# patngnw/NewsRecommendation

Measured on AMD Instinct MI355X. Metric: train impressions/sec @ batch 512, NRMS, higher is better.
Workload: dtype bf16; 1 GPU; NRMS train step (fwd+bwd+Adam), MIND-small shapes: title_len=30, history=50, npratio=4, 300-d word table; per_gpu_batch=512, global_batch=512, vocab_rows=30000, freeze_embedding=False, compact_history=False, dense_batch=False, feed=resident, deterministic=False, optimizer=flat bucket + HIP fused Adam, parallelism=dp1

## Files before the change

newsrecommendation_amd/csrc/nr_api.hip:

```cpp
#include <stdarg.h>
#include <stdio.h>
#include <stdlib.h>
#include <string.h>

#include "nr_gemm.h"

int nr_launch_attn(bool bwd, int dtype, const void* qkv, const float* mask, void* y, const void* dy, void* dqkv, int n, int L,
                   int heads, int d_head, const DropCfg& drop, hipStream_t stream, const uint32_t* tmask = nullptr,
                   const float* bias = nullptr, const int32_t* seq_list = nullptr, const int32_t* seq_count = nullptr,
                   const int32_t* needed = nullptr);
bool nr_attn_pad_ok(int dtype, int L, int d_head, const void* p0, const void* p1);
bool nr_attn_rowsub_ok(int dtype, int L, int d_head, int heads);
bool nr_attn_compact_ok(int dtype, int L, int d_head, int heads);
int nr_launch_attn_bwd_compact(const void* qkv, const float* mask, const void* dy, void* dqkv, int n, int L, int heads, int d_head,
                               const DropCfg& drop, hipStream_t stream, const uint32_t* tmask, const float* bias, const int32_t* seq_list,
                               const int32_t* seq_count, const int32_t* pos, void* dump, float* db, const int32_t* nzf);
int nr_launch_attn_gather_fwd(const void* proj_table, const int32_t* ids, const float* mask, void* y, int n, int L, int heads,
                              int d_head, const DropCfg& drop, hipStream_t stream);
int nr_launch_pool_core_fwd(int dtype, const void* x, const void* e, const float* w2, const float* b2, const float* mask,
                            float* alpha, float* out, int ld_out, int n, int L, int N, int q, hipStream_t s,
                            const int32_t* needed = nullptr);
int nr_launch_pool_core_bwd(int dtype, const void* x, const void* e, const float* w2, const float* alpha, const float* g,
                            int ld_g, void* dpre, float* partial, float* dw2, float* db2, int n, int L, int N, int q,
                            hipStream_t s, const int32_t* seq_nz = nullptr);
// ... 939 lines not shown
  NR_CHECK_ARG(d != nullptr, "additive_pool: null descriptor");
  NR_CHECK_ARG(dtype_ok(d->dtype), "additive_pool: bad dtype %d", d->dtype);
  const int ch = nr_chunk(d->dtype);
  NR_CHECK_ARG(d->n >= 0 && d->L >= 1 && d->L <= 128 && d->N >= 1 && d->q >= 1, "additive_pool: bad shape n=%d L=%d N=%d q=%d", d->n, d->L,
               d->N, d->q);
  NR_CHECK_ARG(d->N % ch == 0 && d->q % ch == 0, "additive_pool: N=%d and q=%d must be multiples of %d for this dtype", d->N, d->q, ch);
  NR_CHECK_ARG(d->ldw1 >= d->N, "additive_pool: ldw1=%d < N=%d", d->ldw1, d->N);
  NR_CHECK_ARG(d->n == 0 || (d->x && d->w1 && d->b1 && d->w2 && d->b2), "additive_pool: null operand");
  return NR_OK;
}

int nr_additive_pool_fwd(const nr_pool_desc* d, void* e, float* alpha, float* out, int ld_out, nr_stream_t stream) {
  int rc = pool_check(d);
  if (rc) return rc;
  if (d->n == 0) return NR_OK;
  NR_CHECK_ARG(e && alpha && out && ld_out >= d->N, "additive_pool_fwd: null output / ld_out");
  NR_DEVICE_GUARD(stream, out);
  hipStream_t s = (hipStream_t)stream;
  if (nr_pool_fused_fwd_ok(d->dtype, d->n, d->L, d->N, d->q, d->ldw1) && ((((uintptr_t)d->x) | ((uintptr_t)d->w1) | ((uintptr_t)e)) & 15) == 0 &&
      d->N % 8 == 0 && d->mask == nullptr)
    return nr_launch_pool_fused_fwd(d->x, d->N, d->w1, d->ldw1, d->b1, d->w2, d->b2, d->mask, e, d->q, alpha, out, ld_out, d->n, d->L, d->N, d->q,
                                    d->seq_needed, s);
  RowSrc A = dense_rows(d->x, d->N, d->N);
  EpiArgs ep = store_epi(e, d->q, d->dtype, d->b1, 1);
  ep.seq_nz = d->seq_needed; ep.L = d->L;
  if ((rc = nr_launch_gemm_nt(d->dtype, A, d->w1, d->ldw1, d->n * d->L, d->q, d->N, EPI_STORE, ep, s))) return rc;
  return nr_launch_pool_core_fwd(d->dtype, d->x, e, d->w2, d->b2, d->mask, alpha, out, ld_out, d->n, d->L, d->N, d->q, s, d->seq_needed);
}

int nr_additive_pool_bwd(const nr_pool_desc* d, const void* e, const float* alpha, const float* g, int ld_g, const void* w1_t,
                         int ldw1t, void* dpre, float* partial, float* dw1, float* db1, float* dw2, float* db2, void* dx,
                         nr_stream_t stream) {
  int rc = pool_check(d);
  if (rc) return rc;
  if (d->n == 0) return NR_OK;
  NR_CHECK_ARG(e && alpha && g && dpre && partial && dw1 && db1 && dw2 && db2, "additive_pool_bwd: null operand");
  NR_DEVICE_GUARD(stream, dpre);
  NR_CHECK_ARG(d->partial_bytes >= pool_ws_elems(d->n, d->L, d->q, d->N, d->dtype) * sizeof(float),
               "additive_pool_bwd: partial holds %zu bytes, nr_pool_workspace_bytes() asks for %zu", d->partial_bytes,
               pool_ws_elems(d->n, d->L, d->q, d->N, d->dtype) * sizeof(float));
  float* tn_scratch = partial + pool_ws_ints(d->n, d->L, d->q);
  const size_t tn_floats = pool_tn_floats(d->n, d->L, d->q, d->N, d->dtype);
  hipStream_t s = (hipStream_t)stream;
  const int M = d->n * d->L;
  DetScope det(s);
  det.add(dw1, (size_t)d->q * d->N);
  det.add(db1, (size_t)d->q);
  det.add(dw2, (size_t)d->q);
  det.add(db2, 1);
  if ((rc = det.begin(true, true))) return rc;
  int32_t* ws = nullptr;
  if (pool_has_flags(d)) {
    ws = reinterpret_cast<int32_t*>(partial + pool_ws_used(d->n, d->q));
    if ((rc = nr_launch_row_flags_f32(g, ld_g, d->N, d->n, ws, s))) return rc;
  }
  const int32_t* zero_flags = ws != nullptr ? ws : d->seq_needed;
  if (ws != nullptr && dx != nullptr && w1_t != nullptr && !det.on() && nr_pool_fused_bwd_ok(d->dtype, d->n, d->L, d->N, d->q, ldw1t) && ld_g % 4 == 0 &&
      ((((uintptr_t)d->x) | ((uintptr_t)e) | ((uintptr_t)w1_t) | ((uintptr_t)dpre) | ((uintptr_t)dx) | ((uintptr_t)g)) & 15) == 0 && d->N % 8 == 0) {
    int rows = 0;
    if ((rc = nr_launch_pool_fused_bwd(d->x, d->N, e, d->q, alpha, g, ld_g, d->w2, w1_t, ldw1t, dpre, d->q, dx, d->N, partial,
                                       nr_pool_partial_rows(d->n), ws, d->n, d->L, d->N, d->q, s, &rows, d->dx_far_unwritten)))
      return rc;
    if ((rc = nr_launch_colsum_split(partial, rows, d->q + 1, d->q + 1, dw2, d->q, db2, s))) return rc;
    if ((rc = nr_launch_live_slabs(ws, d->n, d->L, s))) return rc;
    return gemm_tn_live_slabs(ws, d->n, dpre, d->q, d->x, d->N, dw1, d->N, db1, M, d->q, d->N, d->q, d->N, s, 0, tn_scratch, tn_floats);
  }
  if ((rc = nr_launch_pool_core_bwd(d->dtype, d->x, e, d->w2, alpha, g, ld_g, dpre, partial, dw2, db2, d->n, d->L, d->N, d->q, s, zero_flags)))
    return rc;
  RowSrc X = dense_rows(d->x, d->N, d->N);
  if (ws != nullptr) {
    if ((rc = nr_launch_live_slabs(ws, d->n, d->L, s))) return rc;
    if ((rc = gemm_tn_live_slabs(ws, d->n, dpre, d->q, d->x, d->N, dw1, d->N, db1, M, d->q, d->N, d->q, d->N, s, 0, tn_scratch, tn_floats))) return rc;
  } else if ((rc = nr_launch_gemm_tn(d->dtype, dpre, d->q, X, dw1, d->N, db1, M, d->q, d->N, d->q, d->N, s))) {
    return rc;
  }
  if (dx != nullptr) {
    NR_CHECK_ARG(w1_t != nullptr && ldw1t >= d->q, "additive_pool_bwd: w1_t [N, >=q] needed for dx");
    RowSrc P = dense_rows(dpre, d->q, d->q);
    EpiArgs ep = store_epi(dx, d->N, d->dtype, nullptr, 0);
    ep.rowscale = alpha; ep.G = g; ep.ldg = ld_g; ep.L = d->L;
    ep.seq_nz = zero_flags;
    rc = nr_launch_gemm_nt(d->dtype, P, w1_t, ldw1t, M, d->N, d->q, EPI_POOLBWD, ep, s);
  }
  return rc;
}

static int linear_rows(const nr_linear_desc* d, RowSrc* out) {
  NR_CHECK_ARG(d != nullptr, "linear: null descriptor");
  NR_CHECK_ARG(dtype_ok(d->dtype), "linear: bad dtype %d", d->dtype);
  const int ch = nr_chunk(d->dtype);
  NR_CHECK_ARG(d->M >= 0 && d->K >= 1 && d->N >= 1, "linear: bad shape M=%d K=%d N=%d", d->M, d->K, d->N);
  NR_CHECK_ARG(d->ldx >= round_up(d->K, ch) && d->ldw >= round_up(d->K, ch), "linear: ldx=%d / ldw=%d must cover K=%d rounded up to %d",
               d->ldx, d->ldw, d->K, ch);
  NR_CHECK_ARG(d->M == 0 || (d->x && d->w), "linear: null operand");
  RowSrc s = dense_rows(d->x, d->ldx, d->K);
  if (d->src_kind == NR_SRC_GATHER) {
    NR_CHECK_ARG(d->ids != nullptr && d->ids_stride >= 1, "linear: gather source without ids");
    s.kind = ROWS_GATHER; s.ids = d->ids; s.ids_stride = d->ids_stride;
  } else {
    NR_CHECK_ARG(d->src_kind == NR_SRC_DENSE, "linear: bad src_kind %d", d->src_kind);
  }
  *out = s;
  return NR_OK;
}

int nr_linear_fwd(const nr_linear_desc* d, float* out, int ld_out, nr_stream_t stream) {
  RowSrc A;
  int rc = linear_rows(d, &A);
  if (rc) return rc;
  if (d->M == 0) return NR_OK;
  NR_CHECK_ARG(out != nullptr && ld_out >= d->N, "linear_fwd: null output / ld_out");
  NR_DEVICE_GUARD(stream, out);
  EpiArgs ep = store_epi(out, ld_out, NR_F32, d->bias, 0);
  return nr_launch_gemm_nt(d->dtype, A, d->w, d->ldw, d->M, d->N, round_up(d->K, nr_chunk(d->dtype)), EPI_STORE, ep, (hipStream_t)stream);
}

int nr_linear_bwd(const nr_linear_desc* d, const float* dout, int ld_dout, void* dout_ws, float* dw, float* db, float* dtable,
                  nr_stream_t stream) {
  RowSrc A;
  int rc = linear_rows(d, &A);
  if (rc) return rc;
  if (d->M == 0) return NR_OK;
  NR_CHECK_ARG(dout && dout_ws && dw && db, "linear_bwd: null operand");
  NR_DEVICE_GUARD(stream, dw);
// ... 27 lines not shown
```

newsrecommendation_amd/csrc/nr_gemm.h:

```cpp
#pragma once
#include "nr_common.h"

enum { ROWS_DENSE = 0, ROWS_GATHER = 1, ROWS_IM2COL3 = 2 };

struct RowSrc {
  const void* base;
  const int32_t* ids;
  int ld;
  int ids_stride;
  int kind;
  int Tlen;
  int Dtrue;
  DropCfg drop;
  int gap;
};

enum {
  EPI_STORE = 0,
  EPI_POOLBWD = 1,
  EPI_SCATTER = 2,
  EPI_STORE_TANH = 3,
};

struct EpiArgs {
  void* C;
  int ldc;
  int out_dtype;
  const float* bias;
  int act_tanh;
  const float* rowscale;
  const float* G;
  int ldg, L;
  const int32_t* ids;
  int ids_stride;
  int Dtrue;
  DropCfg drop;
  const int32_t* row_count;
  const int32_t* row_idx;
  const int32_t* row_ids;
  const int32_t* seq_nz;
  void* rows_out;
  int ld_rows_out;
  int a_gap;
  const int32_t* a_idx;
  int a_dense;
  int tail_cus;
};

int nr_launch_gemm_nt(int dtype, const RowSrc& A, const void* B, int ldb, int M, int N, int K, int epi,
                      const EpiArgs& ep, hipStream_t stream);
int nr_launch_conv_rows(int dtype, const RowSrc& A, void* out, int n, hipStream_t stream, const int32_t* needed = nullptr, int margin = 0);
int nr_launch_rows_materialize(int dtype, const RowSrc& A, void* out, int ldo, int M, int K, hipStream_t stream,
                               const int32_t* needed = nullptr, int margin = 0, int L = 0, const int32_t* keep_all = nullptr);
int nr_launch_compact_rows(const int32_t* ids, int ids_stride, int M, int32_t* ws, hipStream_t stream);
int nr_launch_sort_rows_by_id(const int32_t* count, const int32_t* rows, const int32_t* ids, int Mmax, int table_rows, int32_t* hist,
                              int32_t* rows_out, int32_t* ids_out, hipStream_t stream, int32_t* k_out = nullptr,
                              int32_t* counted_cursor = nullptr);
int nr_launch_compact_rows_fwd(const int32_t* ids, int M, int n, int L, const void* table_row0, int cols, int32_t* ws,
                               hipStream_t stream, int32_t* posmap = nullptr, int32_t* zero4 = nullptr, int32_t* zhist = nullptr,
                               int nhist = 0);
int nr_launch_bias_rows(void* C, int ldc, int N, const float* bias, const int32_t* rows, const int32_t* count, int max_rows,
                        const uint32_t* tmask, int L, hipStream_t stream);
int nr_launch_title_flags(const void* dy, int n, int L, int N, int32_t* title_nz, hipStream_t stream);
int nr_launch_row_flags_f32(const float* g, int ld, int N, int n, int32_t* nz, hipStream_t stream);
int nr_launch_live_slabs(int32_t* ws, int n, int L, hipStream_t stream);
int nr_launch_needed_list(const int32_t* flags, int n, int32_t* out, void* y, size_t seq_bytes, hipStream_t stream, int reach = -1,
                          bool zeroed = false);
int nr_launch_seq_list(const int32_t* title_nz, const uint32_t* tmask, int n, int L, int32_t* out, hipStream_t stream, int reach = -1,
                       bool zeroed = false);
int nr_launch_zero_tail_rows(void* buf, int ld, const int32_t* count, int Mmax, hipStream_t stream, int32_t* za = nullptr, int na = 0,
                             int32_t* zb = nullptr, int nb = 0);
int nr_launch_gemm_tn_slabs(const void* dC, int ldc, const void* X, int ldx, float* dW, int ldw, float* db, int M, int N, int K,
                            int Nstore, int Kstore, const int32_t* slab_list, const int32_t* slab_count, hipStream_t stream, int xgap = 0,
                            float* scratch = nullptr, size_t scratch_floats = 0);
size_t nr_gemm_tn_scratch_floats(int M, int N, int K);
bool nr_gemm_tn_slabs_ok(int ldc, int ldx, int M, int N, int K);
int nr_pool_fused_fwd_ok(int dtype, int n, int L, int N, int q, int ldw1);
int nr_launch_pool_fused_fwd(const void* x, int ldx, const void* w1, int ldw1, const float* b1, const float* w2, const float* b2,
                             const float* mask, void* e, int lde, float* alpha, float* out, int ld_out, int n, int L, int N, int q,
                             const int32_t* needed, hipStream_t stream);
int nr_launch_gemm_tn_counted(const void* dC, int ldc, const void* X, int ldx, float* dW, int ldw, int Mmax, int N, int K, int Nstore,
                              int Kstore, const int32_t* row_count, hipStream_t stream, float* scratch = nullptr, size_t scratch_floats = 0);
int nr_pool_fused_bwd_ok(int dtype, int n, int L, int N, int q, int ldw1t);
int nr_launch_pool_fused_bwd(const void* x, int ldx, const void* e, int lde, const float* alpha, const float* g, int ldg, const float* w2,
                             const void* w1t, int ldw1t, void* dpre, int ldp, void* dx, int lddx, float* partial, int partial_rows,
                             const int32_t* nz, int n, int L, int N, int q, hipStream_t stream, int* grid_out, int dx_far_unwritten = 0);
int nr_launch_gather_live_rows(int dtype, const RowSrc& A, void* out, int ldo, int Mmax, int K, const int32_t* count, const int32_t* rows,
                               const int32_t* ids, hipStream_t stream, int32_t* hist = nullptr, int V = 0);
int nr_launch_gemm_tn(int dtype, const void* dC, int ldc, const RowSrc& A, float* dW, int ldw, float* db,
                      int M, int N, int K, int Nstore, int Kstore, hipStream_t stream);
int nr_launch_conv_table_live(const int32_t* ids, int ids_stride, const int32_t* seq_nz, int n, int T, int V, int32_t* hdr, int32_t* live_s,
                              int32_t* live_id, hipStream_t stream);
int nr_launch_conv_table_stage(int dtype, const void* dy, int n, int T, int N, const int32_t* hdr, const int32_t* live_s, bool compact, void* out,
                               int32_t* ident, hipStream_t stream);
int nr_launch_conv_table_rank(const int32_t* hdr, const int32_t* sort_s, const int32_t* sort_id, const int32_t* sort_k, const int32_t* cursor,
                              bool compact, int n, int32_t* ord_s, int32_t* ord_slot, hipStream_t stream);
int nr_launch_conv_table_scatter(int dx_dtype, const void* dx, int ldx, int n, int T, int D, int V, const int32_t* hdr, const int32_t* sort_id,
                                 const int32_t* cursor, const int32_t* ord_s, const int32_t* ord_slot, DropCfg drop, float* dtable,
                                 hipStream_t stream);
```

newsrecommendation_amd/csrc/nr_gemm.hip:

```cpp
#include <stdlib.h>

#include "nr_gemm.h"
#include "nr_scatter_tail.h"

namespace {

constexpr int BM = 128, BN = 128, BK = 32, NTHR = 256;
constexpr int SC = BN + 4;

template <typename T> struct TileCfg {
  static constexpr int CH = 16 / (int)sizeof(T);
  static constexpr int SK = BK + CH;
  static constexpr int CPR = BK / CH;
  static constexpr int NCH = BM * CPR / NTHR;
  static constexpr int RPC = BM / CH;
  static constexpr size_t STAGE_BYTES = (size_t)2 * 2 * BM * SK * sizeof(T);
};
constexpr size_t EPI_BYTES = (size_t)64 * SC * sizeof(float);

template <typename T> constexpr size_t smem_bytes() {
  return TileCfg<T>::STAGE_BYTES > EPI_BYTES ? TileCfg<T>::STAGE_BYTES : EPI_BYTES;
}

union Chunk {
// ... 3280 lines not shown
      for (int u = 0; u < 8; ++u) {
        const int t = base + u * 1024 + tid;
        if (t < n) sFlag[t] = v[u] != 0 ? 1 : 0;
      }
    }
    __syncthreads();
  }
  const int per = (nslab + 1023) / 1024, s0 = tid * per, s1 = min(nslab, s0 + per);
  const int tq = s0 < nslab ? (32 * s0) / L : 0, rq = 32 * s0 - tq * L;
  auto flag = [&](int t) { return in_lds ? (int)sFlag[t] : (title_nz[t] != 0 ? 1 : 0); };
  auto walk = [&](auto&& emit) {
    int t = tq, rem = rq;
    for (int s = s0; s < s1; ++s) {
      int lv = flag(min(t, n - 1)), e = rem + 31, te = t;
      while (e >= L) {
        e -= L; ++te;
        if (te < n) lv |= flag(te);
      }
      emit(s, lv != 0);
      rem += 32;
      while (rem >= L) { rem -= L; ++t; }
    }
  };
  int c = 0;
  walk([&](int, bool lv) { c += lv ? 1 : 0; });
  const int lane = tid & 63, wv = tid >> 6;
  int v = c;
#pragma unroll
  for (int o = 1; o < 64; o <<= 1) {
    const int t = __shfl_up(v, o, 64);
    if (lane >= o) v += t;
  }
  if (lane == 63) sCnt[wv] = v;
  __syncthreads();
  if (wv == 0) {
    int w = lane < 16 ? sCnt[lane] : 0;
#pragma unroll
    for (int o = 1; o < 16; o <<= 1) {
      const int t = __shfl_up(w, o, 64);
      if (lane >= o) w += t;
    }
    if (lane < 16) sCnt[16 + lane] = w;
  }
  __syncthreads();
  int pos = v - c + (wv > 0 ? sCnt[16 + wv - 1] : 0);
  walk([&](int s, bool lv) { if (lv) list[pos++] = s; });
  if (tid == 1023) sCnt[1023] = sCnt[16 + 15];
  if (tid == 1023) *count = sCnt[1023];
}
}

namespace {
__global__ __launch_bounds__(256) void slab_flags_kernel(const int32_t* __restrict__ title_nz, int n, int L, int nslab,
                                                         unsigned char* __restrict__ flags) {
  const int s = blockIdx.x * 256 + threadIdx.x;
  if (s >= nslab) return;
  const int t0 = (32 * s) / L, t1 = min(n - 1, (32 * s + 31) / L);
  bool lv = false;
  for (int t = t0; t <= t1; ++t) lv |= title_nz[t] != 0;
  flags[s] = lv ? 1 : 0;
}
__global__ __launch_bounds__(1024) void slab_list_kernel(const unsigned char* __restrict__ flags, int nslab, int32_t* __restrict__ count,
                                                         int32_t* __restrict__ list) {
  __shared__ int sCnt[32];
  extern __shared__ __attribute__((aligned(16))) unsigned char sFlag[];
  const int tid = threadIdx.x, lane = tid & 63, wv = tid >> 6;
  const int words = (nslab + 3) / 4;
  const uint32_t* fw = reinterpret_cast<const uint32_t*>(flags);
  for (int base = 0; base < words; base += 8 * 1024) {
    uint32_t v[8];
#pragma unroll
    for (int u = 0; u < 8; ++u) {
      const int w = base + u * 1024 + tid;
      v[u] = w < words ? fw[w] : 0u;
    }
#pragma unroll
    for (int u = 0; u < 8; ++u) {
      const int w = base + u * 1024 + tid;
      if (w < words) reinterpret_cast<uint32_t*>(sFlag)[w] = v[u];
    }
  }
  __syncthreads();
  const int per = (nslab + 1023) / 1024, s0 = tid * per, s1 = min(nslab, s0 + per);
  int c = 0;
  for (int s2 = s0; s2 < s1; ++s2) c += sFlag[s2];
  int v = c;
#pragma unroll
  for (int o = 1; o < 64; o <<= 1) {
    const int t = __shfl_up(v, o, 64);
    if (lane >= o) v += t;
  }
  if (lane == 63) sCnt[wv] = v;
  __syncthreads();
  if (wv == 0) {
    int w = lane < 16 ? sCnt[lane] : 0;
#pragma unroll
    for (int o = 1; o < 16; o <<= 1) {
      const int t = __shfl_up(w, o, 64);
      if (lane >= o) w += t;
    }
    if (lane < 16) sCnt[16 + lane] = w;
  }
  __syncthreads();
  int pos = v - c + (wv > 0 ? sCnt[16 + wv - 1] : 0);
  for (int s2 = s0; s2 < s1; ++s2)
    if (sFlag[s2]) list[pos++] = s2;
  if (tid == 0) *count = sCnt[16 + 15];
}
// ... 97 lines not shown
}
__global__ __launch_bounds__(256) void zero_unneeded_kernel(const int32_t* __restrict__ flags, uint4* __restrict__ y, int chunks16, int n,
                                                            int reach) {
  const int seq = blockIdx.x;
  if (flags[seq] != 0) return;
  if (reach >= 0) {
    bool near = false;
    for (int t = max(0, seq - reach) + (int)threadIdx.x; t <= min(n - 1, seq + reach); t += 256) near |= flags[t] != 0;
    if (!__syncthreads_or(near)) return;
  }
  uint4* p = y + (size_t)seq * chunks16;
  for (int c = threadIdx.x; c < chunks16; c += 256) p[c] = make_uint4(0, 0, 0, 0);
}
}
int nr_launch_needed_list(const int32_t* flags, int n, int32_t* out, void* y, size_t seq_bytes, hipStream_t stream, int reach, bool zeroed) {
  NR_CHECK_ARG(flags != nullptr && out != nullptr && y != nullptr && seq_bytes % 16 == 0 && (((uintptr_t)y) & 15) == 0, "needed_list: bad arguments");
  if (!zeroed) NR_CHECK_HIP(hipMemsetAsync(out, 0, 4 * sizeof(int32_t), stream));
  NrProfScope ps(stream, "needed_list[n=%d]", n);
  hipLaunchKernelGGL(needed_list_kernel, dim3((n + 255) / 256), dim3(256), 0, stream, flags, n, out, out + 4);
  hipLaunchKernelGGL(zero_unneeded_kernel, dim3(n), dim3(256), 0, stream, flags, reinterpret_cast<uint4*>(y), (int)(seq_bytes / 16), n, reach);
  NR_CHECK_LAUNCH();
  return NR_OK;
}

int nr_launch_seq_list(const int32_t* title_nz, const uint32_t* tmask, int n, int L, int32_t* out, hipStream_t stream, int reach, bool zeroed) {
  if (!zeroed) NR_CHECK_HIP(hipMemsetAsync(out, 0, 4 * sizeof(int32_t), stream));
  hipLaunchKernelGGL(seq_list_kernel, dim3((n + 255) / 256), dim3(256), 0, stream, title_nz, tmask, n, reach >= 0 ? reach : 32 / L + 2, out,
                     out + 4);
  NR_CHECK_LAUNCH();
  return NR_OK;
}

namespace {
__global__ __launch_bounds__(256) void zero_tail_rows_kernel(uint4* __restrict__ buf, int chunks, const int32_t* __restrict__ count, int Mmax,
                                                             int32_t* __restrict__ za, int na, int32_t* __restrict__ zb, int nb) {
  const int t = blockIdx.x * 256 + threadIdx.x, stride = gridDim.x * 256;
  for (int i = t; i < na; i += stride) za[i] = 0;
  for (int i = t; i < nb; i += stride) zb[i] = 0;
  if (blockIdx.x != 0) return;
  const int n = *count, end = min(Mmax, (n + 31) / 32 * 32);
  for (int u = threadIdx.x; u < (end - n) * chunks; u += 256) buf[(size_t)n * chunks + u] = make_uint4(0, 0, 0, 0);
}
}
int nr_launch_zero_tail_rows(void* buf, int ld, const int32_t* count, int Mmax, hipStream_t stream, int32_t* za, int na, int32_t* zb, int nb) {
  NR_CHECK_ARG(buf != nullptr && count != nullptr && ld % 8 == 0 && (((uintptr_t)buf) & 15) == 0, "zero_tail_rows: bad arguments");
  if (za == nullptr) na = 0;
  if (zb == nullptr) nb = 0;
  const int most = na > nb ? na : nb, grid = most > 4096 ? 16 : 1;
  hipLaunchKernelGGL(zero_tail_rows_kernel, dim3(grid), dim3(256), 0, stream, (uint4*)buf, ld / 8, count, Mmax, za, na, zb, nb);
  NR_CHECK_LAUNCH();
  return NR_OK;
}

int nr_launch_live_slabs(int32_t* ws, int n, int L, hipStream_t stream) {
  const int M = n * L, nslab = M / 32;
  NR_CHECK_ARG(ws != nullptr && M % 32 == 0, "live_slabs: bad arguments");
  int32_t* list = ws + n + 4;
  if (nslab >= 4 && nslab <= 128 * 1024) {
    unsigned char* flags = reinterpret_cast<unsigned char*>(list + nslab - (nslab + 3) / 4);
    hipLaunchKernelGGL(slab_flags_kernel, dim3((nslab + 255) / 256), dim3(256), 0, stream, ws, n, L, nslab, flags);
    hipLaunchKernelGGL(slab_list_kernel, dim3(1), dim3(1024), (size_t)((nslab + 15) / 16) * 16, stream, flags, nslab, ws + n, list);
    NR_CHECK_LAUNCH();
    return NR_OK;
  }
  const int in_lds = n <= 128 * 1024 ? 1 : 0;
  hipLaunchKernelGGL(live_slabs_kernel, dim3(1), dim3(1024), in_lds ? (size_t)((n + 15) / 16) * 16 : 0, stream, ws, n, L, nslab, ws + n,
                     list, in_lds);
  NR_CHECK_LAUNCH();
  return NR_OK;
}

int nr_launch_gemm_tn_slabs(const void* dC, int ldc, const void* X, int ldx, float* dW, int ldw, float* db, int M, int N, int K,
                            int Nstore, int Kstore, const int32_t* slab_list, const int32_t* slab_count, hipStream_t stream, int xgap,
                            float* scratch, size_t scratch_floats) {
  NR_CHECK_ARG(tn3::eligible(ldc, ldx, M, N, K), "gemm_tn_slabs: shape not eligible");
  NrProfScope ps(stream, "gemm_tn3_live[bf16,Mmax=%d,N=%d,K=%d,gap=%d]", M, N, K, xgap);
  return tn3::launch(dC, ldc, X, ldx, dW, ldw, db, M, N, K, Nstore, Kstore, stream, slab_list, slab_count, xgap, scratch, scratch_floats);
}
size_t nr_gemm_tn_scratch_floats(int M, int N, int K) { return tn3::scratch_floats(M, N, K); }
bool nr_gemm_tn_slabs_ok(int ldc, int ldx, int M, int N, int K) { return tn3::eligible(ldc, ldx, M, N, K); }
int nr_launch_gemm_tn_counted(const void* dC, int ldc, const void* X, int ldx, float* dW, int ldw, int Mmax, int N, int K, int Nstore,
                              int Kstore, const int32_t* row_count, hipStream_t stream, float* scratch, size_t scratch_floats) {
  NR_CHECK_ARG(tn3::eligible(ldc, ldx, Mmax, N, K) && row_count != nullptr, "gemm_tn_counted: shape not eligible");
  NrProfScope ps(stream, "gemm_tn3_rows[bf16,Mmax=%d,N=%d,K=%d,gap=0]", Mmax, N, K);
  return tn3::launch(dC, ldc, X, ldx, dW, ldw, nullptr, Mmax, N, K, Nstore, Kstore, stream, nullptr, row_count, 0, scratch, scratch_floats);
}

int nr_launch_gemm_tn(int dtype, const void* dC, int ldc, const RowSrc& A, float* dW, int ldw, float* db, int M, int N,
                      int K, int Nstore, int Kstore, hipStream_t stream) {
  const int ch = nr_chunk(dtype);
  NR_CHECK_ARG(M > 0 && N > 0 && K > 0, "gemm_tn: empty problem M=%d N=%d K=%d", M, N, K);
  NR_CHECK_ARG(N % ch == 0 && K % ch == 0 && ldc % ch == 0 && A.ld % ch == 0, "gemm_tn: N=%d K=%d ldc=%d lda=%d must be multiples of %d",
               N, K, ldc, A.ld, ch);
  NR_CHECK_ARG(((uintptr_t)A.base & 15) == 0 && ((uintptr_t)dC & 15) == 0, "gemm_tn: operands must be 16-byte aligned");
  if (dtype == NR_BF16 && A.kind == ROWS_DENSE && A.drop.thresh == 0) {
    if (tn3::eligible(ldc, A.ld, M, N, K)) {
      NrProfScope ps(stream, "gemm_tn3[bf16,M=%d,N=%d,K=%d,gap=%d]", M, N, K, A.gap);
      return tn3::launch(dC, ldc, A.base, A.ld, dW, ldw, db, M, N, K, Nstore, Kstore, stream, nullptr, nullptr, A.gap);
    }
    if (A.gap == 0) {
      NrProfScope ps(stream, "gemm_tn2[bf16,M=%d,N=%d,K=%d]", M, N, K);
      return tn2::launch(dC, ldc, A.base, A.ld, dW, ldw, db, M, N, K, Nstore, Kstore, stream);
    }
  }
  NrProfScope ps(stream, "gemm_tn[%s,rows=%d,M=%d,N=%d,K=%d]", dtype == NR_BF16 ? "bf16" : "f32", A.kind, M, N, K);
  return dtype == NR_BF16 ? launch_tn_d<bf16_t>(dC, ldc, A, dW, ldw, db, M, N, K, Nstore, Kstore, stream)
                          : launch_tn_d<float>(dC, ldc, A, dW, ldw, db, M, N, K, Nstore, Kstore, stream);
}
```

newsrecommendation_amd/csrc/nr_pool.hip:

```cpp
#include "nr_common.h"

namespace {

template <typename T> struct ChunkOf { static constexpr int CH = 16 / (int)sizeof(T); };
template <typename T> __device__ __forceinline__ void load_chunk_f(const T* p, float (&f)[ChunkOf<T>::CH]);
template <> __device__ __forceinline__ void load_chunk_f<float>(const float* p, float (&f)[4]) {
  const f32x4 v = *reinterpret_cast<const f32x4*>(p);
  f[0] = v[0]; f[1] = v[1]; f[2] = v[2]; f[3] = v[3];
}
template <> __device__ __forceinline__ void load_chunk_f<bf16_t>(const bf16_t* p, float (&f)[8]) {
  const bf16x8 v = *reinterpret_cast<const bf16x8*>(p);
#pragma unroll
  for (int e = 0; e < 8; ++e) f[e] = (float)v[e];
}
template <typename T> __device__ __forceinline__ void store_chunk_f(T* p, const float (&f)[ChunkOf<T>::CH]);
template <> __device__ __forceinline__ void store_chunk_f<float>(float* p, const float (&f)[4]) {
  *reinterpret_cast<f32x4*>(p) = (f32x4){f[0], f[1], f[2], f[3]};
}
template <> __device__ __forceinline__ void store_chunk_f<bf16_t>(bf16_t* p, const float (&f)[8]) {
  bf16x8 v;
#pragma unroll
  for (int e = 0; e < 8; ++e) v[e] = (bf16_t)f[e];
  *reinterpret_cast<bf16x8*>(p) = v;
}

template <typename T>
__device__ __forceinline__ float wave_row_dot(const T* __restrict__ row, const float* __restrict__ vec, int nchunks, int lane) {
  constexpr int CH = ChunkOf<T>::CH;
  float p = 0.f;
  for (int c = lane; c < nchunks; c += 64) {
    float f[CH];
    load_chunk_f<T>(row + c * CH, f);
#pragma unroll
    for (int e = 0; e < CH; ++e) p = fmaf(f[e], vec[c * CH + e], p);
  }
  return wave_sum(p);
}

constexpr int POOL_RED_FLOATS = 256 * 8;

template <typename T, int TPL = 1>
__global__ __launch_bounds__(256) void pool_fwd_kernel(const T* __restrict__ x, const T* __restrict__ e,
                                                       const float* __restrict__ w2, const float* __restrict__ b2,
                                                       const float* __restrict__ mask, float* __restrict__ alpha,
                                                       float* __restrict__ out, int ld_out, int L, int N, int q,
                                                       const int32_t* __restrict__ needed) {
  constexpr int CH = ChunkOf<T>::CH;
  __shared__ float sS[64 * TPL];
  __shared__ float sRed[POOL_RED_FLOATS];
  const int seq = blockIdx.x, tid = threadIdx.x, lane = tid & 63, wid = __builtin_amdgcn_readfirstlane(tid >> 6);
  const size_t row0 = (size_t)seq * L;
  if (needed != nullptr && needed[seq] == 0) {
    for (int l = tid; l < L; l += 256) alpha[row0 + l] = 0.f;
// ... 250 lines not shown
    for (int r = r0; r < r1; ++r) {
      const float d = (float)dout[(size_t)r * N + c];
      const float m = mask ? mask[r] : 1.f;
      dx[(size_t)r * N + c] = d * m;
      acc = fmaf(1.f - m, d, acc);
    }
    if (mask && dpad) nr_accum(dpad + c, acc, nr_fix_on());
  }
}

template <typename T>
__global__ __launch_bounds__(256) void blend_bwd4_kernel(const T* __restrict__ dout, const float* __restrict__ mask,
                                                         float* __restrict__ dx, float* __restrict__ dpad, int rows,
                                                         int N, int rows_per_block) {
  extern __shared__ float sAcc[];
  const int cg = N / 4, rl_n = 256 / cg;
  const int tid = threadIdx.x, rl = tid / cg, c = (tid - rl * cg) * 4;
  const int r0 = blockIdx.x * rows_per_block, r1 = min(rows, r0 + rows_per_block);
  float acc[4] = {0.f, 0.f, 0.f, 0.f};
  if (rl < rl_n) {
    for (int r = r0 + rl; r < r1; r += rl_n) {
      float d[4];
      if (sizeof(T) == 2) {
        const bf16x4 v = *reinterpret_cast<const bf16x4*>(dout + (size_t)r * N + c);
#pragma unroll
        for (int e = 0; e < 4; ++e) d[e] = (float)v[e];
      } else {
        const f32x4 v = *reinterpret_cast<const f32x4*>(dout + (size_t)r * N + c);
#pragma unroll
        for (int e = 0; e < 4; ++e) d[e] = v[e];
      }
      const float m = mask ? mask[r] : 1.f;
      f32x4 o;
#pragma unroll
      for (int e = 0; e < 4; ++e) { o[e] = d[e] * m; acc[e] = fmaf(1.f - m, d[e], acc[e]); }
      *reinterpret_cast<f32x4*>(dx + (size_t)r * N + c) = o;
    }
  }
  if (mask && dpad) {
    if (rl < rl_n) {
#pragma unroll
      for (int e = 0; e < 4; ++e) sAcc[rl * N + c + e] = acc[e];
    }
    __syncthreads();
    const bool det = nr_fix_on();
    for (int k = tid; k < N; k += 256) {
      float t = 0.f;
      for (int j = 0; j < rl_n; ++j) t += sAcc[j * N + k];
      nr_accum(dpad + k, t, det);
    }
  }
}

__global__ __launch_bounds__(64) void score_ce_fwd_kernel(const float* __restrict__ cand, int ld_cand,
                                                          const float* __restrict__ user,
                                                          const int64_t* __restrict__ label, float* __restrict__ score,
                                                          float* __restrict__ lossvec, int C, int N) {
  const int b = blockIdx.x, lane = threadIdx.x;
  const float* u = user + (size_t)b * N;
  float my = -INFINITY;
  for (int j0 = 0; j0 < C; j0 += 8) {
    float p[8] = {0.f, 0.f, 0.f, 0.f, 0.f, 0.f, 0.f, 0.f};
    for (int c = lane; c < N; c += 64) {
      const float uc = u[c];
#pragma unroll
      for (int t = 0; t < 8; ++t)
        if (j0 + t < C) p[t] = fmaf(cand[((size_t)b * C + j0 + t) * ld_cand + c], uc, p[t]);
    }
#pragma unroll
    for (int t = 0; t < 8; ++t) {
      const float q = wave_sum(p[t]);
      if (lane == j0 + t) my = q;
    }
  }
  if (lane < C) score[(size_t)b * C + lane] = my;
  const float m = wave_max(my);
  const float ex = lane < C ? expf(my - m) : 0.f;
  const float lse = m + logf(wave_sum(ex));
  const int lab = (int)label[b];
  const float sl = __shfl(my, lab, 64);
  if (lane == 0) lossvec[b] = lse - sl;
}

__global__ __launch_bounds__(256) void mean_kernel(const float* __restrict__ v, int n, float* __restrict__ out) {
  __shared__ float red[256];
  float s = 0.f;
  for (int i = threadIdx.x; i < n; i += 256) s += v[i];
  red[threadIdx.x] = s;
  __syncthreads();
  for (int o = 128; o > 0; o >>= 1) {
    if (threadIdx.x < o) red[threadIdx.x] += red[threadIdx.x + o];
    __syncthreads();
  }
  if (threadIdx.x == 0) out[0] = red[0] / (float)n;
}

__global__ __launch_bounds__(256) void score_ce_bwd_kernel(const float* __restrict__ cand, int ld_cand,
                                                           const float* __restrict__ user,
                                                           const int64_t* __restrict__ label,
                                                           const float* __restrict__ score,
                                                           const float* __restrict__ gloss,
                                                           const float* __restrict__ gscore, float inv_b,
                                                           float* __restrict__ dcand, int ld_dcand,
                                                           float* __restrict__ duser, int C, int N) {
  __shared__ float sD[64];
  const int b = blockIdx.x, tid = threadIdx.x;
  if (tid < 64) {
    const float s = tid < C ? score[(size_t)b * C + tid] : -INFINITY;
    const float m = wave_max(s);
    const float ex = tid < C ? expf(s - m) : 0.f;
    const float sum = wave_sum(ex);
    if (tid < C) {
      float d = (ex / sum - (tid == (int)label[b] ? 1.f : 0.f)) * (gloss ? gloss[0] * inv_b : 0.f);
      if (gscore) d += gscore[(size_t)b * C + tid];
      sD[tid] = d;
    }
  }
  __syncthreads();
  for (int c = tid; c < N; c += 256) {
    const float u = user[(size_t)b * N + c];
    float du = 0.f;
    for (int j = 0; j < C; ++j) {
      const float d = sD[j];
      dcand[((size_t)b * C + j) * ld_dcand + c] = d * u;
      du = fmaf(d, cand[((size_t)b * C + j) * ld_cand + c], du);
    }
    duser[(size_t)b * N + c] = du;
  }
}

__global__ __launch_bounds__(256) void score_eval_kernel(const float* __restrict__ news, int ld_news,
                                                         const int32_t* __restrict__ cand_ids,
                                                         const int32_t* __restrict__ imp_of,
                                                         const float* __restrict__ user, int ld_user,
                                                         float* __restrict__ score, int n_cand, int N) {
  const int i = blockIdx.x * 4 + (threadIdx.x >> 6), lane = threadIdx.x & 63;
  if (i >= n_cand) return;
  const float* nr = news + (size_t)cand_ids[i] * ld_news;
  const float* u = user + (size_t)imp_of[i] * ld_user;
  float p = 0.f;
  if (((N | ld_news | ld_user) & 3) == 0 && ((((uintptr_t)news) | ((uintptr_t)user)) & 15) == 0) {
    for (int c = 4 * lane; c < N; c += 256) {
      const f32x4 a = *reinterpret_cast<const f32x4*>(nr + c), b = *reinterpret_cast<const f32x4*>(u + c);
      p = fmaf(a[0], b[0], fmaf(a[1], b[1], fmaf(a[2], b[2], fmaf(a[3], b[3], p))));
    }
  } else {
    for (int c = lane; c < N; c += 64) p = fmaf(nr[c], u[c], p);
// ... 353 lines not shown
  NR_DEVICE_GUARD(stream, out);
  if (n_ids == 0) return NR_OK;
  NR_CHECK_ARG(n_ids > 0 && cols > 0 && ld_out >= cols && ld_table >= cols, "gather_cast_fwd: bad sizes");
  NrProfScope ps((hipStream_t)stream, "gather_cast[n=%d,cols=%d]", n_ids, cols);
  hipLaunchKernelGGL(gather_cast_kernel, dim3((n_ids + 3) / 4), dim3(256), 0, (hipStream_t)stream, table, ld_table, ids, n_ids, cols, (bf16_t*)out, ld_out);
  NR_CHECK_LAUNCH();
  return NR_OK;
}

int nr_embed_gather_bwd(const float* dout, int ld_dout, const int32_t* ids, int n_ids, int ids_stride, int cols,
                        float* dtable, int ld_dtable, nr_stream_t stream) {
  NR_CHECK_ARG(dout && ids && dtable, "embed_gather_bwd: null pointer");
  NR_DEVICE_GUARD(stream, dtable);
  if (n_ids == 0) return NR_OK;
  hipLaunchKernelGGL(gather_bwd_kernel, dim3((n_ids + 3) / 4), dim3(256), 0, (hipStream_t)stream, dout, ld_dout, ids, n_ids, ids_stride, cols, dtable, ld_dtable);
  NR_CHECK_LAUNCH();
  return NR_OK;
}

int nr_pad_blend_fwd(const float* x, const float* mask, const float* pad, void* out, int n, int L, int N, int dtype,
                     nr_stream_t stream) {
  NR_CHECK_ARG(x && out && n > 0 && L > 0 && N > 0, "pad_blend_fwd: null/empty");
  NR_CHECK_ARG(mask == nullptr || pad != nullptr, "pad_blend_fwd: mask without pad_doc");
  NR_DEVICE_GUARD(stream, out);
  const size_t rows = (size_t)n * L;
  hipStream_t s = (hipStream_t)stream;
  NrProfScope ps(s, "pad_blend_fwd[n=%d,L=%d,N=%d]", n, L, N);
  if (N % 4 == 0 && rows * (size_t)(N / 4) < (1ull << 31) && (((uintptr_t)x | (uintptr_t)out | (uintptr_t)pad) & 15) == 0) {
    const uint32_t N4 = (uint32_t)(N / 4);
    const dim3 grid(grid_for(rows * N4));
    if (dtype == NR_BF16) hipLaunchKernelGGL(blend_fwd4_kernel<bf16_t>, grid, dim3(256), 0, s, x, mask, pad, (bf16_t*)out, (uint32_t)rows, N4);
    else hipLaunchKernelGGL(blend_fwd4_kernel<float>, grid, dim3(256), 0, s, x, mask, pad, (float*)out, (uint32_t)rows, N4);
    NR_CHECK_LAUNCH();
    return NR_OK;
  }
  if (dtype == NR_BF16)
    hipLaunchKernelGGL(blend_fwd_kernel<bf16_t>, dim3(grid_for(rows * N)), dim3(256), 0, s, x, mask, pad, (bf16_t*)out, rows, N);
  else
    hipLaunchKernelGGL(blend_fwd_kernel<float>, dim3(grid_for(rows * N)), dim3(256), 0, s, x, mask, pad, (float*)out, rows, N);
  NR_CHECK_LAUNCH();
  return NR_OK;
}

int nr_pad_blend_bwd(const void* dout, const float* mask, float* dx, float* dpad, int n, int L, int N, int dtype,
                     nr_stream_t stream) {
  NR_CHECK_ARG(dout && dx && n > 0 && L > 0 && N > 0, "pad_blend_bwd: null/empty");
  NR_DEVICE_GUARD(stream, dx);
  const int rows = n * L, rpb = 32;
  hipStream_t s = (hipStream_t)stream;
  int det_rc = NR_OK;
  const int det = (mask != nullptr && dpad != nullptr) ? nr_det_open(s, dpad, (size_t)N, nullptr, 0, false, true, &det_rc) : 0;
  if (det_rc) return det_rc;
  NrProfScope ps(s, "pad_blend_bwd[n=%d,L=%d,N=%d]", n, L, N);
  if (N % 4 == 0 && N / 4 <= 256 && (((uintptr_t)dout | (uintptr_t)dx) & 15) == 0) {
    const int rl_n = 256 / (N / 4), rpb4 = 64;
    const size_t smem = (size_t)rl_n * N * sizeof(float);
    if (dtype == NR_BF16)
      hipLaunchKernelGGL(blend_bwd4_kernel<bf16_t>, dim3((rows + rpb4 - 1) / rpb4), dim3(256), smem, s, (const bf16_t*)dout, mask, dx, dpad, rows, N, rpb4);
    else
      hipLaunchKernelGGL(blend_bwd4_kernel<float>, dim3((rows + rpb4 - 1) / rpb4), dim3(256), smem, s, (const float*)dout, mask, dx, dpad, rows, N, rpb4);
    NR_CHECK_LAUNCH();
    return nr_det_close(det);
  }
  if (dtype == NR_BF16)
    hipLaunchKernelGGL(blend_bwd_kernel<bf16_t>, dim3((rows + rpb - 1) / rpb), dim3(256), 0, s, (const bf16_t*)dout, mask, dx, dpad, rows, N, rpb);
  else
    hipLaunchKernelGGL(blend_bwd_kernel<float>, dim3((rows + rpb - 1) / rpb), dim3(256), 0, s, (const float*)dout, mask, dx, dpad, rows, N, rpb);
  NR_CHECK_LAUNCH();
  return nr_det_close(det);
}

int nr_score_ce_fwd(const float* cand, int ld_cand, const float* user, const int64_t* label, float* score, float* loss,
                    float* lossvec, int B, int C, int N, nr_stream_t stream) {
  NR_CHECK_ARG(cand && user && label && score && loss && lossvec, "score_ce_fwd: null pointer");
  NR_CHECK_ARG(B > 0 && C >= 1 && C <= 64 && N > 0, "score_ce_fwd: B=%d C=%d (1..64) N=%d", B, C, N);
  NR_DEVICE_GUARD(stream, score);
  hipStream_t s = (hipStream_t)stream;
  NrProfScope ps(s, "score_ce_fwd[B=%d,C=%d,N=%d]", B, C, N);
  hipLaunchKernelGGL(score_ce_fwd_kernel, dim3(B), dim3(64), 0, s, cand, ld_cand, user, label, score, lossvec, C, N);
  hipLaunchKernelGGL(mean_kernel, dim3(1), dim3(256), 0, s, lossvec, B, loss);
  NR_CHECK_LAUNCH();
  return NR_OK;
}

int nr_score_ce_bwd(const float* cand, int ld_cand, const float* user, const int64_t* label, const float* score,
                    const float* gloss, const float* gscore, float* dcand, int ld_dcand, float* duser, int B, int C, int N,
                    nr_stream_t stream) {
  NR_CHECK_ARG(cand && user && label && score && dcand && duser, "score_ce_bwd: null pointer");
  NR_CHECK_ARG(B > 0 && C >= 1 && C <= 64 && N > 0, "score_ce_bwd: B=%d C=%d (1..64) N=%d", B, C, N);
  NR_DEVICE_GUARD(stream, dcand);
  NrProfScope ps((hipStream_t)stream, "score_ce_bwd[B=%d,C=%d,N=%d]", B, C, N);
  hipLaunchKernelGGL(score_ce_bwd_kernel, dim3(B), dim3(256), 0, (hipStream_t)stream, cand, ld_cand, user, label, score, gloss, gscore, 1.0f / (float)B, dcand, ld_dcand, duser, C, N);
  NR_CHECK_LAUNCH();
  return NR_OK;
}

int nr_score_eval(const float* news_vecs, int ld_news, const int32_t* cand_ids, const int32_t* imp_of, const float* user,
                  int ld_user, float* score, int n_cand, int N, nr_stream_t stream) {
  NR_CHECK_ARG(news_vecs && cand_ids && imp_of && user && score, "score_eval: null pointer");
  NR_DEVICE_GUARD(stream, score);
  if (n_cand == 0) return NR_OK;
  hipLaunchKernelGGL(score_eval_kernel, dim3((n_cand + 3) / 4), dim3(256), 0, (hipStream_t)stream, news_vecs, ld_news, cand_ids, imp_of, user, ld_user, score, n_cand, N);
  NR_CHECK_LAUNCH();
  return NR_OK;
}

int nr_dropout_mask(float* out, uint32_t count, float p, uint32_t seed, nr_stream_t stream) {
  NR_CHECK_ARG(out != nullptr, "dropout_mask: null pointer");
  NR_DEVICE_GUARD(stream, out);
  if (count == 0) return NR_OK;
  const DropCfg d = nr_make_drop(p, seed);
  hipLaunchKernelGGL(dropout_mask_kernel, dim3(grid_for(count)), dim3(256), 0, (hipStream_t)stream, out, count, d.key, d.thresh);
  NR_CHECK_LAUNCH();
  return NR_OK;
}

}
```

Measured before the change: 178,600 impressions/s.

## Fuse score/CE mean, widen pad-blend backward, reuse seq flags in pool backward

The score/CE forward now handles four batch rows per block and computes the loss mean in its last block through a ticket counter, so the separate mean kernel launch goes away. Pad-blend backward gains a 1024-thread kernel sized to one block per CU for the non-deterministic path. Additive-pool backward reuses the existing seq_needed flags instead of recomputing row flags, and copies them into the workspace inside the slab-flags kernel. These are several small launch and bandwidth reductions; the global ticket slots add cross-launch state and a possible race if more than 64 calls are in flight at once.

```diff
diff --git a/newsrecommendation_amd/csrc/nr_api.hip b/newsrecommendation_amd/csrc/nr_api.hip
--- a/newsrecommendation_amd/csrc/nr_api.hip
+++ b/newsrecommendation_amd/csrc/nr_api.hip
@@ -1015,24 +1015,25 @@
   int32_t* ws = nullptr;
   if (pool_has_flags(d)) {
     ws = reinterpret_cast<int32_t*>(partial + pool_ws_used(d->n, d->q));
-    if ((rc = nr_launch_row_flags_f32(g, ld_g, d->N, d->n, ws, s))) return rc;
-  }
-  const int32_t* zero_flags = ws != nullptr ? ws : d->seq_needed;
+    if (d->seq_needed == nullptr && (rc = nr_launch_row_flags_f32(g, ld_g, d->N, d->n, ws, s))) return rc;
+  }
+  const int32_t* zero_flags = d->seq_needed != nullptr ? d->seq_needed : ws;
+  const int32_t* copy_from = ws != nullptr ? d->seq_needed : nullptr;
   if (ws != nullptr && dx != nullptr && w1_t != nullptr && !det.on() && nr_pool_fused_bwd_ok(d->dtype, d->n, d->L, d->N, d->q, ldw1t) && ld_g % 4 == 0 &&
       ((((uintptr_t)d->x) | ((uintptr_t)e) | ((uintptr_t)w1_t) | ((uintptr_t)dpre) | ((uintptr_t)dx) | ((uintptr_t)g)) & 15) == 0 && d->N % 8 == 0) {
     int rows = 0;
     if ((rc = nr_launch_pool_fused_bwd(d->x, d->N, e, d->q, alpha, g, ld_g, d->w2, w1_t, ldw1t, dpre, d->q, dx, d->N, partial,
-                                       nr_pool_partial_rows(d->n), ws, d->n, d->L, d->N, d->q, s, &rows, d->dx_far_unwritten)))
+                                       nr_pool_partial_rows(d->n), zero_flags, d->n, d->L, d->N, d->q, s, &rows, d->dx_far_unwritten)))
       return rc;
     if ((rc = nr_launch_colsum_split(partial, rows, d->q + 1, d->q + 1, dw2, d->q, db2, s))) return rc;
-    if ((rc = nr_launch_live_slabs(ws, d->n, d->L, s))) return rc;
+    if ((rc = nr_launch_live_slabs(ws, d->n, d->L, s, copy_from))) return rc;
     return gemm_tn_live_slabs(ws, d->n, dpre, d->q, d->x, d->N, dw1, d->N, db1, M, d->q, d->N, d->q, d->N, s, 0, tn_scratch, tn_floats);
   }
   if ((rc = nr_launch_pool_core_bwd(d->dtype, d->x, e, d->w2, alpha, g, ld_g, dpre, partial, dw2, db2, d->n, d->L, d->N, d->q, s, zero_flags)))
     return rc;
   RowSrc X = dense_rows(d->x, d->N, d->N);
   if (ws != nullptr) {
-    if ((rc = nr_launch_live_slabs(ws, d->n, d->L, s))) return rc;
+    if ((rc = nr_launch_live_slabs(ws, d->n, d->L, s, copy_from))) return rc;
     if ((rc = gemm_tn_live_slabs(ws, d->n, dpre, d->q, d->x, d->N, dw1, d->N, db1, M, d->q, d->N, d->q, d->N, s, 0, tn_scratch, tn_floats))) return rc;
   } else if ((rc = nr_launch_gemm_tn(d->dtype, dpre, d->q, X, dw1, d->N, db1, M, d->q, d->N, d->q, d->N, s))) {
     return rc;
diff --git a/newsrecommendation_amd/csrc/nr_gemm.h b/newsrecommendation_amd/csrc/nr_gemm.h
--- a/newsrecommendation_amd/csrc/nr_gemm.h
+++ b/newsrecommendation_amd/csrc/nr_gemm.h
@@ -63,7 +63,7 @@
                         const uint32_t* tmask, int L, hipStream_t stream);
 int nr_launch_title_flags(const void* dy, int n, int L, int N, int32_t* title_nz, hipStream_t stream);
 int nr_launch_row_flags_f32(const float* g, int ld, int N, int n, int32_t* nz, hipStream_t stream);
-int nr_launch_live_slabs(int32_t* ws, int n, int L, hipStream_t stream);
+int nr_launch_live_slabs(int32_t* ws, int n, int L, hipStream_t stream, const int32_t* src = nullptr);
 int nr_launch_needed_list(const int32_t* flags, int n, int32_t* out, void* y, size_t seq_bytes, hipStream_t stream, int reach = -1,
                           bool zeroed = false);
 int nr_launch_seq_list(const int32_t* title_nz, const uint32_t* tmask, int n, int L, int32_t* out, hipStream_t stream, int reach = -1,
diff --git a/newsrecommendation_amd/csrc/nr_gemm.hip b/newsrecommendation_amd/csrc/nr_gemm.hip
--- a/newsrecommendation_amd/csrc/nr_gemm.hip
+++ b/newsrecommendation_amd/csrc/nr_gemm.hip
@@ -3356,8 +3356,9 @@
 
 namespace {
 __global__ __launch_bounds__(256) void slab_flags_kernel(const int32_t* __restrict__ title_nz, int n, int L, int nslab,
-                                                         unsigned char* __restrict__ flags) {
+                                                         unsigned char* __restrict__ flags, int32_t* __restrict__ copy) {
   const int s = blockIdx.x * 256 + threadIdx.x;
+  if (copy != nullptr && s < n) copy[s] = title_nz[s] != 0 ? 1 : 0;
   if (s >= nslab) return;
   const int t0 = (32 * s) / L, t1 = min(n - 1, (32 * s + 31) / L);
   bool lv = false;
@@ -3561,17 +3562,20 @@
   return NR_OK;
 }
 
-int nr_launch_live_slabs(int32_t* ws, int n, int L, hipStream_t stream) {
+int nr_launch_live_slabs(int32_t* ws, int n, int L, hipStream_t stream, const int32_t* src) {
   const int M = n * L, nslab = M / 32;
   NR_CHECK_ARG(ws != nullptr && M % 32 == 0, "live_slabs: bad arguments");
   int32_t* list = ws + n + 4;
   if (nslab >= 4 && nslab <= 128 * 1024) {
     unsigned char* flags = reinterpret_cast<unsigned char*>(list + nslab - (nslab + 3) / 4);
-    hipLaunchKernelGGL(slab_flags_kernel, dim3((nslab + 255) / 256), dim3(256), 0, stream, ws, n, L, nslab, flags);
+    const int threads = src != nullptr && n > nslab ? n : nslab;
+    hipLaunchKernelGGL(slab_flags_kernel, dim3((threads + 255) / 256), dim3(256), 0, stream, src != nullptr ? src : (const int32_t*)ws, n, L, nslab,
+                       flags, src != nullptr ? ws : (int32_t*)nullptr);
     hipLaunchKernelGGL(slab_list_kernel, dim3(1), dim3(1024), (size_t)((nslab + 15) / 16) * 16, stream, flags, nslab, ws + n, list);
     NR_CHECK_LAUNCH();
     return NR_OK;
   }
+  if (src != nullptr) NR_CHECK_HIP(hipMemcpyAsync(ws, src, (size_t)n * sizeof(int32_t), hipMemcpyDeviceToDevice, stream));
   const int in_lds = n <= 128 * 1024 ? 1 : 0;
   hipLaunchKernelGGL(live_slabs_kernel, dim3(1), dim3(1024), in_lds ? (size_t)((n + 15) / 16) * 16 : 0, stream, ws, n, L, nslab, ws + n,
                      list, in_lds);
diff --git a/newsrecommendation_amd/csrc/nr_pool.hip b/newsrecommendation_amd/csrc/nr_pool.hip
--- a/newsrecommendation_amd/csrc/nr_pool.hip
+++ b/newsrecommendation_amd/csrc/nr_pool.hip
@@ -1,4 +1,5 @@
 #include "nr_common.h"
+#include <atomic>
 
 namespace {
 
@@ -355,47 +356,147 @@
   }
 }
 
-__global__ __launch_bounds__(64) void score_ce_fwd_kernel(const float* __restrict__ cand, int ld_cand,
-                                                          const float* __restrict__ user,
-                                                          const int64_t* __restrict__ label, float* __restrict__ score,
-                                                          float* __restrict__ lossvec, int C, int N) {
-  const int b = blockIdx.x, lane = threadIdx.x;
-  const float* u = user + (size_t)b * N;
-  float my = -INFINITY;
-  for (int j0 = 0; j0 < C; j0 += 8) {
-    float p[8] = {0.f, 0.f, 0.f, 0.f, 0.f, 0.f, 0.f, 0.f};
-    for (int c = lane; c < N; c += 64) {
-      const float uc = u[c];
-#pragma unroll
-      for (int t = 0; t < 8; ++t)
-        if (j0 + t < C) p[t] = fmaf(cand[((size_t)b * C + j0 + t) * ld_cand + c], uc, p[t]);
-    }
-#pragma unroll
-    for (int t = 0; t < 8; ++t) {
-      const float q = wave_sum(p[t]);
-      if (lane == j0 + t) my = q;
-    }
-  }
-  if (lane < C) score[(size_t)b * C + lane] = my;
-  const float m = wave_max(my);
-  const float ex = lane < C ? expf(my - m) : 0.f;
-  const float lse = m + logf(wave_sum(ex));
-  const int lab = (int)label[b];
-  const float sl = __shfl(my, lab, 64);
-  if (lane == 0) lossvec[b] = lse - sl;
-}
-
-__global__ __launch_bounds__(256) void mean_kernel(const float* __restrict__ v, int n, float* __restrict__ out) {
+template <typename T, int W>
+__global__ __launch_bounds__(1024) void blend_bwdw_kernel(const T* __restrict__ dout, const float* __restrict__ mask,
+                                                          float* __restrict__ dx, float* __restrict__ dpad, int rows,
+                                                          int N, int rows_per_block) {
+  constexpr int U = 4;
+  extern __shared__ float sAcc[];
+  const int cg = N / W, rl_n = 1024 / cg;
+  const int tid = threadIdx.x, rl = tid / cg, c = (tid - rl * cg) * W;
+  const int r0 = blockIdx.x * rows_per_block, r1 = min(rows, r0 + rows_per_block);
+  float acc[W];
+#pragma unroll
+  for (int e = 0; e < W; ++e) acc[e] = 0.f;
+  if (rl < rl_n) {
+    for (int r = r0 + rl; r < r1; r += U * rl_n) {
+      float d[U][W], m[U];
+#pragma unroll
+      for (int u = 0; u < U; ++u) {
+        const int rr = r + u * rl_n;
+        if (rr < r1) {
+          const T* p = dout + (size_t)rr * N + c;
+          if (sizeof(T) == 2) {
+            if (W == 8) {
+              const bf16x8 v = *reinterpret_cast<const bf16x8*>(p);
+#pragma unroll
+              for (int e = 0; e < W; ++e) d[u][e] = (float)v[e];
+            } else {
+              const bf16x4 v = *reinterpret_cast<const bf16x4*>(p);
+#pragma unroll
+              for (int e = 0; e < W; ++e) d[u][e] = (float)v[e];
+            }
+          } else {
+#pragma unroll
+            for (int h = 0; h < W / 4; ++h) {
+              const f32x4 v = *reinterpret_cast<const f32x4*>(p + 4 * h);
+#pragma unroll
+              for (int e = 0; e < 4; ++e) d[u][4 * h + e] = v[e];
+            }
+          }
+          m[u] = mask ? mask[rr] : 1.f;
+        }
+      }
+#pragma unroll
+      for (int u = 0; u < U; ++u) {
+        const int rr = r + u * rl_n;
+        if (rr < r1) {
+#pragma unroll
+          for (int h = 0; h < W / 4; ++h) {
+            f32x4 o;
+#pragma unroll
+            for (int e = 0; e < 4; ++e) {
+              o[e] = d[u][4 * h + e] * m[u];
+              acc[4 * h + e] = fmaf(1.f - m[u], d[u][4 * h + e], acc[4 * h + e]);
+            }
+            *reinterpret_cast<f32x4*>(dx + (size_t)rr * N + c + 4 * h) = o;
+          }
+        }
+      }
+    }
+  }
+  if (mask && dpad) {
+    if (rl < rl_n) {
+#pragma unroll
+      for (int e = 0; e < W; ++e) sAcc[rl * N + c + e] = acc[e];
+    }
+    __syncthreads();
+    const bool det = nr_fix_on();
+    for (int k = tid; k < N; k += 1024) {
+      float t = 0.f;
+      for (int j = 0; j < rl_n; ++j) t += sAcc[j * N + k];
+      nr_accum(dpad + k, t, det);
+    }
+  }
+}
+
+constexpr int NR_SCORE_TICKETS = 64;
+__device__ unsigned int g_score_ticket[NR_SCORE_TICKETS];
+
+__global__ __launch_bounds__(256) void score_ce_fwd_kernel(const float* __restrict__ cand, int ld_cand,
+                                                           const float* __restrict__ user,
+                                                           const int64_t* __restrict__ label, float* __restrict__ score,
+                                                           float* lossvec, float* __restrict__ loss, int slot, int B, int C, int N) {
   __shared__ float red[256];
+  __shared__ int sLast;
+  const int tid = threadIdx.x, lane = tid & 63, wv = tid >> 6;
+  const int b = blockIdx.x * 4 + wv;
+  if (b < B) {
+    const float* u = user + (size_t)b * N;
+    float my = -INFINITY;
+    for (int j0 = 0; j0 < C; j0 += 8) {
+      float p[8] = {0.f, 0.f, 0.f, 0.f, 0.f, 0.f, 0.f, 0.f};
+      const float* cb = cand + ((size_t)b * C + j0) * ld_cand;
+      for (int c0 = lane; c0 < N; c0 += 4 * 64) {
+        float uc[4], x[8][4];
+#pragma unroll
+        for (int k = 0; k < 4; ++k) {
+          const int c = c0 + 64 * k;
+          uc[k] = c < N ? u[c] : 0.f;
+#pragma unroll
+          for (int t = 0; t < 8; ++t) x[t][k] = (c < N && j0 + t < C) ? cb[(size_t)t * ld_cand + c] : 0.f;
+        }
+#pragma unroll
+        for (int k = 0; k < 4; ++k) {
+          if (c0 + 64 * k < N) {
+#pragma unroll
+            for (int t = 0; t < 8; ++t)
+              if (j0 + t < C) p[t] = fmaf(x[t][k], uc[k], p[t]);
+          }
+        }
+      }
+#pragma unroll
+      for (int t = 0; t < 8; ++t) {
+        const float q = wave_sum(p[t]);
+        if (lane == j0 + t) my = q;
+      }
+    }
+    if (lane < C) score[(size_t)b * C + lane] = my;
+    const float m = wave_max(my);
+    const float ex = lane < C ? expf(my - m) : 0.f;
+    const float lse = m + logf(wave_sum(ex));
+    const int lab = (int)label[b];
+    const float sl = __shfl(my, lab, 64);
+    if (lane == 0) lossvec[b] = lse - sl;
+  }
+  __threadfence();
+  __syncthreads();
+  if (tid == 0) sLast = atomicAdd(&g_score_ticket[slot], 1u) == gridDim.x - 1 ? 1 : 0;
+  __syncthreads();
+  if (sLast == 0) return;
+  __threadfence();
   float s = 0.f;
-  for (int i = threadIdx.x; i < n; i += 256) s += v[i];
-  red[threadIdx.x] = s;
+  for (int i = tid; i < B; i += 256) s += __hip_atomic_load(lossvec + i, __ATOMIC_RELAXED, __HIP_MEMORY_SCOPE_AGENT);
+  red[tid] = s;
   __syncthreads();
   for (int o = 128; o > 0; o >>= 1) {
-    if (threadIdx.x < o) red[threadIdx.x] += red[threadIdx.x + o];
+    if (tid < o) red[tid] += red[tid + o];
     __syncthreads();
   }
-  if (threadIdx.x == 0) out[0] = red[0] / (float)n;
+  if (tid == 0) {
+    loss[0] = red[0] / (float)B;
+    atomicExch(&g_score_ticket[slot], 0u);
+  }
 }
 
 __global__ __launch_bounds__(256) void score_ce_bwd_kernel(const float* __restrict__ cand, int ld_cand,
@@ -855,7 +956,27 @@
   const int det = (mask != nullptr && dpad != nullptr) ? nr_det_open(s, dpad, (size_t)N, nullptr, 0, false, true, &det_rc) : 0;
   if (det_rc) return det_rc;
   NrProfScope ps(s, "pad_blend_bwd[n=%d,L=%d,N=%d]", n, L, N);
-  if (N % 4 == 0 && N / 4 <= 256 && (((uintptr_t)dout | (uintptr_t)dx) & 15) == 0) {
+  const bool aligned16 = (((uintptr_t)dout | (uintptr_t)dx) & 15) == 0;
+  if (det == 0 && N % 4 == 0 && N / 4 <= 256 && aligned16) {
+    static int cus = 0;
+    if (cus == 0) {
+      int dev = 0, c = 0;
+      NR_CHECK_HIP(hipGetDevice(&dev));
+      NR_CHECK_HIP(hipDeviceGetAttribute(&c, hipDeviceAttributeMultiprocessorCount, dev));
+      cus = c >= 8 ? c : 256;
+    }
+    const int rl_n = 1024 / (N / 4), round = 4 * rl_n;
+    const int rpb = ((rows + cus - 1) / cus + round - 1) / round * round;
+    const dim3 grid((rows + rpb - 1) / rpb);
+    const size_t smem = (size_t)rl_n * N * sizeof(float);
+    if (dtype == NR_BF16)
+      hipLaunchKernelGGL((blend_bwdw_kernel<bf16_t, 4>), grid, dim3(1024), smem, s, (const bf16_t*)dout, mask, dx, dpad, rows, N, rpb);
+    else
+      hipLaunchKernelGGL((blend_bwdw_kernel<float, 4>), grid, dim3(1024), smem, s, (const float*)dout, mask, dx, dpad, rows, N, rpb);
+    NR_CHECK_LAUNCH();
+    return nr_det_close(det);
+  }
+  if (N % 4 == 0 && N / 4 <= 256 && aligned16) {
     const int rl_n = 256 / (N / 4), rpb4 = 64;
     const size_t smem = (size_t)rl_n * N * sizeof(float);
     if (dtype == NR_BF16)
@@ -880,8 +1001,9 @@
   NR_DEVICE_GUARD(stream, score);
   hipStream_t s = (hipStream_t)stream;
   NrProfScope ps(s, "score_ce_fwd[B=%d,C=%d,N=%d]", B, C, N);
-  hipLaunchKernelGGL(score_ce_fwd_kernel, dim3(B), dim3(64), 0, s, cand, ld_cand, user, label, score, lossvec, C, N);
-  hipLaunchKernelGGL(mean_kernel, dim3(1), dim3(256), 0, s, lossvec, B, loss);
+  static std::atomic<unsigned> next_slot{0};
+  const int slot = (int)(next_slot.fetch_add(1u) % (unsigned)NR_SCORE_TICKETS);
+  hipLaunchKernelGGL(score_ce_fwd_kernel, dim3((B + 3) / 4), dim3(256), 0, s, cand, ld_cand, user, label, score, lossvec, loss, slot, B, C, N);
   NR_CHECK_LAUNCH();
   return NR_OK;
 }
```

Measured after the change: 180,000 impressions/s, median of 6. No clear change (+0.8%).
